# yifanlu0227/CoAlign

Hardware: AMD Instinct MI355X
Metric: frames_per_s_5agent_opv2v_synthetic (higher is better)
Workload: dtype f32 (3x3 convolutions: every operand rounded to 22 significant bits and split into two fp16 terms, the low term scaled by 2^10 and the weights by a per-output-channel power of two so that both terms are normal fp16 numbers at any scale; three fp16 matrix products per fp32 product, f32 accumulation

## Files before the change

### coalign_amd/csrc/conv3x3_sp_s2.hip

```cpp
#include "common.h"

namespace {

typedef float floatx16 __attribute__((ext_vector_type(16)));
typedef _Float16 halfx8 __attribute__((ext_vector_type(8)));
typedef __attribute__((address_space(3))) void *lptr_t;

constexpr int kCoutTile = 64;
constexpr int TH = 4, TW = 32;
constexpr int PR = 2 * TH + 1;
constexpr int CPP = 34, ROWP = 2 * CPP;
constexpr int PIX = PR * ROWP, PIXP = (PIX + 63) / 64 * 64, PINS = PIXP / 64;
constexpr int WQ = 9 * 2 * 2 * kCoutTile, WINS = WQ / 64;
constexpr int W_BYTES = WQ * 16, B_BYTES = 4 * PIXP * 16;
constexpr int kMaxCout = 1024, kMaxCoutSkip = 512;
constexpr size_t OPERAND_BYTES = 2 * (size_t)W_BYTES + 2 * (size_t)B_BYTES, LDS_BYTES = OPERAND_BYTES + 2 * kMaxCout * sizeof(float);
constexpr int WAVES = 8, THREADS = 64 * WAVES;
constexpr int WJ = 5, PJ = 2, OPS = WJ + 4 * PJ;
static_assert(LDS_BYTES <= 160 * 1024, "LDS budget");
static_assert(PINS == 10 && WINS == 36, "the piece schedule below is written for 10 patch and 36 weight instructions");

struct S2Args {
    const uint4 *__restrict__ x;
    const unsigned long long *__restrict__ stamps;
    const int *__restrict__ tag_ptr;
    unsigned sparse_rows;
    const uint4 *__restrict__ wt, *__restrict__ zero;
    const float *__restrict__ bias, *__restrict__ wscale;
    uint4 *__restrict__ y;
    const uint4 *__restrict__ ws;
    const float *__restrict__ ws_scale;
    float *__restrict__ yskip;
    int *range_flag;
    int N, Cin, Cout, H, W, Ho, Wo, relu, tiles_x, tiles_y, total_tasks;
    int ablate;
#ifdef COALIGN_LAB
    long long *trace;
#endif
};

#ifdef COALIGN_LAB
#define S2_STAMP(k) if (a.trace && (g == 0 || g == 100) && lane == 0 && L < 64) a.trace[((((g ? 1 : 0) * 8 + wave) * 64) + L) * 4 + (k)] = (long long)__builtin_amdgcn_s_memtime()
#else
#define S2_STAMP(k)
#endif

__device__ __forceinline__ void swap32(unsigned &a, unsigned &b) {
    const auto q = __builtin_amdgcn_permlane32_swap(a, b, false, false);
    const unsigned x = q[0], y = q[1];
    a = x;
    b = y;
}

__device__ __forceinline__ void dma16(const uint4 *src, unsigned lds_byte) {
    asm volatile("s_mov_b32 m0, %0\n\ts_nop 0\n\tglobal_load_lds_dwordx4 %1, off" ::"s"(__builtin_amdgcn_readfirstlane(lds_byte)), "v"(src) : "memory", "m0");
}

struct Task {
    int cg, n, oy0, ox0;
};

struct Plan {
    int off[PJ];
    const uint4 *wsrc;
};

template <bool SPARSE, bool SKIP>
__global__ __launch_bounds__(THREADS, 2) void conv3x3_sp_s2_kernel(const S2Args a) {
    extern __shared__ __attribute__((aligned(1024))) char lds[];
    const int tid = threadIdx.x, wave = __builtin_amdgcn_readfirstlane(tid >> 6), lane = tid & 63, half = lane >> 5, p = lane & 31;
    const int HW = a.H * a.W, HWo = a.Ho * a.Wo, CI16 = a.Cin / 16, CO16 = a.Cout / 16, groups = a.Cout / kCoutTile, chunks = CI16;
    const unsigned lds0 = (unsigned)(size_t)(lptr_t)lds;
    const int bx = wave & 3, cq = wave >> 2;
    const int oyl = p >> 3, oxl = bx * 8 + (p & 7);
    int boff[9];
#pragma unroll
    for (int s = 0; s < 9; ++s) {
        const int dy = s / 3, dx = s % 3;
        boff[s] = 2 * half * PIXP + (2 * oyl + dy) * ROWP + (dx & 1) * CPP + oxl + (dx >> 1);
    }
    const int wlane = half * kCoutTile + cq * 32 + p;
    const unsigned tag = SPARSE ? (unsigned)*a.tag_ptr : 0u;
    float *lds_par = reinterpret_cast<float *>(lds + OPERAND_BYTES);
    for (int i = tid; i < a.Cout / 4; i += THREADS) {
        reinterpret_cast<float4 *>(lds_par)[i] = reinterpret_cast<const float4 *>(a.bias)[i];
        reinterpret_cast<float4 *>(lds_par + a.Cout)[i] = reinterpret_cast<const float4 *>(a.wscale)[i];
        if constexpr (SKIP) reinterpret_cast<float4 *>(lds_par + 2 * a.Cout)[i] = reinterpret_cast<const float4 *>(a.ws_scale)[i];
    }
    auto skip_w = [&](int cg, int c, uint4 (&w)[2]) {
        const uint4 *base = a.ws + ((size_t)(cg * chunks + c) * 4 + half) * kCoutTile + cq * 32 + p;
        w[0] = base[0];
        w[1] = base[2 * kCoutTile];
    };

    auto decode = [&](int t) {
        Task c;
        c.cg = t % groups;
        const int sp = t / groups, ty = sp / a.tiles_x;
        c.ox0 = (sp - ty * a.tiles_x) * TW;
        c.n = ty / a.tiles_y;
        c.oy0 = (ty - c.n * a.tiles_y) * TH;
        return c;
    };
    auto position = [&](const Task &t, int j, int &iy, int &ix) {
        const int ins = j == 0 ? wave : 8 + wave;
        const int i = ins * 64 + lane, r = i / ROWP, rem = i - r * ROWP, cp = rem >= CPP ? 1 : 0, k = rem - cp * CPP;
        iy = 2 * t.oy0 - 1 + r;
        ix = 2 * t.ox0 - 1 + 2 * k + cp;
        return (j == 0 || wave < 2) && i < PIX && k < (cp ? TW : TW + 1) && iy >= 0 && iy < a.H && ix >= 0 && ix < a.W;
    };
    auto make_plan_dense = [&](const Task &t) {
        Plan pl;
        pl.wsrc = a.wt + (size_t)t.cg * chunks * WQ + lane;
#pragma unroll
        for (int j = 0; j < PJ; ++j) {
            int iy, ix;
            const bool ok = position(t, j, iy, ix);
            pl.off[j] = ok ? t.n * CI16 * 4 * HW + iy * a.W + ix : -1;
        }
        return pl;
    };
    struct Stamps {
        unsigned long long st[PJ];
    };
    auto load_stamps = [&](const Task &t) {
        Stamps s;
#pragma unroll
        for (int j = 0; j < PJ; ++j) {
            int iy, ix;
            const bool ok = position(t, j, iy, ix);
            s.st[j] = 0ull;
            if (ok) s.st[j] = a.stamps[((size_t)t.n * a.H + iy) * a.W + ix];
        }
        return s;
    };
    auto make_plan_sparse = [&](const Task &t, const Stamps &s) {
        Plan pl;
        pl.wsrc = a.wt + (size_t)t.cg * chunks * WQ + lane;
#pragma unroll
        for (int j = 0; j < PJ; ++j) {
            const unsigned row = (unsigned)s.st[j];
            const bool ok = (unsigned)(s.st[j] >> 32) == tag && tag != 0u && row < a.sparse_rows;
            pl.off[j] = ok ? (int)(row * (unsigned)(CI16 * 4)) : -1;
        }
        return pl;
    };
    auto issue_op = [&](const Plan &pl, int c, int slot, int k) {
        if (k < WJ) {
            const bool ok = wave < 2 ? k < 3 : true;
            const int piece = wave < 2 ? 3 * wave + k : 6 + 5 * (wave - 2) + k;
            if (ok && !(a.ablate & 1)) dma16(pl.wsrc + (size_t)c * WQ + piece * 64, lds0 + slot * W_BYTES + piece * 1024);
        } else {
            const int j = (k - WJ) / 4, q = (k - WJ) % 4, ins = j == 0 ? wave : 8 + wave;
            if ((j == 0 || wave < 2) && !(a.ablate & 2)) {
                const uint4 *src = pl.off[j] < 0 ? a.zero : SPARSE ? a.x + (size_t)pl.off[j] + (c * 4 + q) : a.x + (size_t)pl.off[j] + ((size_t)c * 4 + q) * HW;
                dma16(src, lds0 + 2 * W_BYTES + slot * B_BYTES + (q * PIXP + ins * 64) * 16);
            }
        }
    };
    auto issue_all = [&](const Plan &pl, int c, int slot) {
#pragma unroll
        for (int k = 0; k < OPS; ++k) issue_op(pl, c, slot, k);
    };

    const int n_wg = gridDim.x;
    int g = blockIdx.x;
    {
        const int q = n_wg >> 3, r = n_wg & 7, k = g & 7, j = g >> 3;
        g = k * q + (k < r ? k : r) + j;
    }
    const int n_local = ((a.total_tasks - g + n_wg - 1) / n_wg) * chunks;
    if (n_local <= 0) return;
    int task = g;
    Task cur = decode(task);
    Plan plan;
    if constexpr (SPARSE) plan = make_plan_sparse(cur, load_stamps(cur));
    else plan = make_plan_dense(cur);
    issue_all(plan, 0, 0);
    if (wave >= WAVES / 2) __builtin_amdgcn_s_setprio(1);
    uint4 sw_cur[2] = {}, sw_nxt[2] = {};
    if constexpr (SKIP) skip_w(cur.cg, 0, sw_nxt);
    int L = 0;
    while (L < n_local) {
        const int oy = cur.oy0 + oyl, ox = cur.ox0 + oxl;
        const bool live = oy < a.Ho && ox < a.Wo;
        const bool wave_live = __builtin_amdgcn_readfirstlane((int)(cur.ox0 + bx * 8 < a.Wo)) != 0;
        const size_t pix = live ? (size_t)oy * a.Wo + ox : 0;
        floatx16 acc = {0}, accl = {0}, sacc = {0}, saccl = {0};
        Task next = cur;
        Plan nplan = plan;
        int ntask = task;
        Stamps nst;
#pragma unroll
        for (int j = 0; j < PJ; ++j) nst.st[j] = 0ull;
        for (int chunk = 0; chunk < chunks; ++chunk, ++L) {
            S2_STAMP(0);
            __builtin_amdgcn_s_waitcnt(0);
            S2_STAMP(1);
            __syncthreads();
            S2_STAMP(2);
            if constexpr (SKIP) {
#pragma unroll
                for (int t = 0; t < 2; ++t) {
                    asm volatile("" : "+v"(sw_nxt[t].x), "+v"(sw_nxt[t].y), "+v"(sw_nxt[t].z), "+v"(sw_nxt[t].w));
                    sw_cur[t] = sw_nxt[t];
                }
            }
            const bool more = L + 1 < n_local;
            int nc = chunk + 1;
            if constexpr (SPARSE) {
                if (chunk == chunks - 2 && L + 2 < n_local) {
                    ntask = task + n_wg;
                    next = decode(ntask);
                    nst = load_stamps(next);
                }
            }
            if (more && nc == chunks) {
                nc = 0;
                if constexpr (SPARSE) {
                    nplan = make_plan_sparse(next, nst);
                } else {
                    ntask = task + n_wg;
                    next = decode(ntask);
                    nplan = make_plan_dense(next);
                }
            }
            if constexpr (SKIP) {
                if (more) skip_w(nc == 0 ? next.cg : cur.cg, nc, sw_nxt);
            }
            const int slot_cur = L & 1, slot_next = (L + 1) & 1;
            if (wave_live && !(a.ablate & 4)) {
                const uint4 *bq = reinterpret_cast<const uint4 *>(lds + 2 * W_BYTES + slot_cur * B_BYTES), *wq = reinterpret_cast<const uint4 *>(lds + slot_cur * W_BYTES) + wlane;
                auto load_b = [&](int s, halfx8 (&b)[2]) {
#pragma unroll
                    for (int t = 0; t < 2; ++t) b[t] = __builtin_bit_cast(halfx8, bq[t * PIXP + boff[s]]);
                };
                auto load_w = [&](int s, halfx8 (&w)[2]) {
#pragma unroll
                    for (int t = 0; t < 2; ++t) w[t] = __builtin_bit_cast(halfx8, wq[((s * 2 + t) * 2) * kCoutTile]);
                };
                halfx8 bc[2], wc[2];
                load_b(0, bc);
                load_w(0, wc);
#pragma unroll
                for (int s = 0; s < 9; ++s) {
                    if (!(a.ablate & 16)) {
                        if (s == 0) __builtin_amdgcn_s_setprio(2);
                        if (s == 3) __builtin_amdgcn_s_setprio(1);
                        if (s == 6) __builtin_amdgcn_s_setprio(0);
                    }
                    halfx8 bn[2], wn[2];
                    if (s + 1 < 9) {
                        load_b(s + 1, bn);
                        load_w(s + 1, wn);
                    }
                    accl = __builtin_amdgcn_mfma_f32_32x32x16_f16(wc[0], bc[1], accl, 0, 0, 0);
                    acc = __builtin_amdgcn_mfma_f32_32x32x16_f16(wc[0], bc[0], acc, 0, 0, 0);
                    accl = __builtin_amdgcn_mfma_f32_32x32x16_f16(wc[1], bc[0], accl, 0, 0, 0);
                    if constexpr (SKIP) {
                        if (s == 4) {
                            const halfx8 sh = __builtin_bit_cast(halfx8, sw_cur[0]), sl = __builtin_bit_cast(halfx8, sw_cur[1]);
                            saccl = __builtin_amdgcn_mfma_f32_32x32x16_f16(sh, bc[1], saccl, 0, 0, 0);
                            sacc = __builtin_amdgcn_mfma_f32_32x32x16_f16(sh, bc[0], sacc, 0, 0, 0);
                            saccl = __builtin_amdgcn_mfma_f32_32x32x16_f16(sl, bc[0], saccl, 0, 0, 0);
                        }
                    }
                    if (more) {
                        if (a.ablate & 32) {
#pragma unroll
                            for (int k = s; k < OPS; k += 9) issue_op(nplan, nc, slot_next, k);
                        } else {
#pragma unroll
                            for (int k = 2 * s; k < 2 * s + 2; ++k)
                                if (k < OPS) issue_op(nplan, nc, slot_next, k);
                        }
                    }
                    if (s + 1 < 9) {
#pragma unroll
                        for (int t = 0; t < 2; ++t) {
                            bc[t] = bn[t];
                            wc[t] = wn[t];
                        }
                    }
                }
            } else if (more) {
                issue_all(nplan, nc, slot_next);
            }
            S2_STAMP(3);
        }
#pragma unroll
        for (int e = 0; e < 16; ++e) acc[e] = fmaf(accl[e], coalign::kSp16LowInv, acc[e]);
        const int ch0 = cur.cg * kCoutTile + cq * 32 + 4 * half;
        const float4 *bias4 = reinterpret_cast<const float4 *>(lds_par + ch0), *winv4 = reinterpret_cast<const float4 *>(lds_par + a.Cout + ch0);
        const float floor_v = a.relu ? 0.f : -__builtin_inff();
        float vmax = 0.f;
        uint4 *ysp = a.y + ((size_t)(cur.n * CO16 + cur.cg * 4 + cq * 2) * 4 + half) * HWo + pix;
        const size_t sp_step = 2 * (size_t)HWo;
#pragma unroll
        for (int g8 = 0; g8 < 4; ++g8) {
            const float4 b4 = bias4[2 * g8], i4 = winv4[2 * g8];
            const float bb[4] = {b4.x, b4.y, b4.z, b4.w}, ii[4] = {i4.x, i4.y, i4.z, i4.w};
            float v[4];
#pragma unroll
            for (int j = 0; j < 4; ++j) v[j] = fmaxf(acc[4 * g8 + j] * ii[j] + (0.f + bb[j]), floor_v);
            vmax = fmaxf(fmaxf(fabsf(v[0]), fabsf(v[1])), fmaxf(fmaxf(fabsf(v[2]), fabsf(v[3])), vmax));
            unsigned h01, l01, h23, l23;
            coalign::sp16_split2(v[0], v[1], h01, l01);
            coalign::sp16_split2(v[2], v[3], h23, l23);
            swap32(h01, l01);
            swap32(h23, l23);
            if (live && wave_live && !(a.ablate & 8)) *ysp = uint4{h01, h23, l01, l23};
            ysp += sp_step;
        }
        if (a.range_flag && live && wave_live && vmax > 65504.f) atomicOr(a.range_flag, 1);
        if constexpr (SKIP) {
            const float4 *sinv4 = reinterpret_cast<const float4 *>(lds_par + 2 * a.Cout + ch0);
            float4 *ys = reinterpret_cast<float4 *>(a.yskip + ((size_t)cur.n * HWo + pix) * a.Cout + ch0);
#pragma unroll
            for (int g8 = 0; g8 < 4; ++g8) {
                const float4 i4 = sinv4[2 * g8];
                float4 o;
                o.x = fmaf(saccl[4 * g8], coalign::kSp16LowInv, sacc[4 * g8]) * i4.x;
                o.y = fmaf(saccl[4 * g8 + 1], coalign::kSp16LowInv, sacc[4 * g8 + 1]) * i4.y;
                o.z = fmaf(saccl[4 * g8 + 2], coalign::kSp16LowInv, sacc[4 * g8 + 2]) * i4.z;
                o.w = fmaf(saccl[4 * g8 + 3], coalign::kSp16LowInv, sacc[4 * g8 + 3]) * i4.w;
                if (live && wave_live && !(a.ablate & 8)) ys[2 * g8] = o;
            }
        }
        cur = next;
        plan = nplan;
        task = ntask;
    }
}

__global__ void sp_pack_rows_kernel(const float *__restrict__ rows, uint4 *__restrict__ out, int M, const int *__restrict__ count_ptr, int C, int *range_flag) {
    const size_t i = (size_t)blockIdx.x * blockDim.x + threadIdx.x;
    const int G8 = C / 8;
    if (count_ptr) M = min(max(*count_ptr, 0), M);
    if (i >= (size_t)M * G8) return;
    const int g8 = (int)(i % G8);
    const size_t row = i / G8;
    const float4 *src = reinterpret_cast<const float4 *>(rows + row * C + 8 * g8);
    const float4 q0 = src[0], q1 = src[1];
    const float v[8] = {q0.x, q0.y, q0.z, q0.w, q1.x, q1.y, q1.z, q1.w};
    unsigned h[4], l[4];
    bool big = false;
#pragma unroll
    for (int k = 0; k < 4; ++k) {
        coalign::sp16_split2(v[2 * k], v[2 * k + 1], h[k], l[k]);
        big = big || fabsf(v[2 * k]) > 65504.f || fabsf(v[2 * k + 1]) > 65504.f;
    }
    const size_t base = row * (size_t)(C / 16 * 4) + (size_t)(g8 / 2) * 4 + (g8 % 2) * 2;
    out[base] = uint4{h[0], h[1], h[2], h[3]};
    out[base + 1] = uint4{l[0], l[1], l[2], l[3]};
    if (range_flag && big) atomicOr(range_flag, 1);
}

#ifdef COALIGN_LAB
long long *g_s2_trace = nullptr;
#endif

int s2_check(int N, int Cin, int Cout, int H, int W) {
    if (N < 0 || H < 1 || W < 1 || Cin < 1 || Cout < 1) return COALIGN_ERR_BAD_SHAPE;
    if (Cin % 16 || Cout % kCoutTile || Cout > kMaxCout) return COALIGN_ERR_UNSUPPORTED;
    if ((int64_t)N * (Cin > Cout ? Cin : Cout) * H * W > (int64_t)1 << 32) return COALIGN_ERR_UNSUPPORTED;
    return COALIGN_OK;
}

template <bool SPARSE, bool SKIP>
int launch_s2(S2Args a, hipStream_t s) {
    constexpr int kMaxDev = 16;
    static int cus[kMaxDev] = {0};
    int dev = 0;
    if (hipGetDevice(&dev) != hipSuccess || dev < 0 || dev >= kMaxDev) dev = 0;
    auto kern = conv3x3_sp_s2_kernel<SPARSE, SKIP>;
    if (!cus[dev]) {
        hipDeviceProp_t prop;
        if (hipGetDeviceProperties(&prop, dev) != hipSuccess || prop.multiProcessorCount <= 0) prop.multiProcessorCount = 256;
        const int rc = coalign::hip_call(hipFuncSetAttribute(reinterpret_cast<const void *>(kern), hipFuncAttributeMaxDynamicSharedMemorySize, (int)LDS_BYTES));
        if (rc != COALIGN_OK) {
            (void)hipGetLastError();
            return rc;
        }
        cus[dev] = prop.multiProcessorCount;
    }
    a.Ho = (a.H + 1) / 2;
    a.Wo = (a.W + 1) / 2;
    a.tiles_x = (a.Wo + TW - 1) / TW;
    a.tiles_y = (a.Ho + TH - 1) / TH;
    a.total_tasks = a.tiles_x * a.tiles_y * a.N * (a.Cout / kCoutTile);
    const int rounds = (a.total_tasks + cus[dev] - 1) / cus[dev], grid = (a.total_tasks + rounds - 1) / rounds;
    hipLaunchKernelGGL(kern, dim3(grid), dim3(THREADS), LDS_BYTES, s, a);
    return coalign::check_launch();
}

int fill_common(S2Args &a, const void *w_split, const float *bias, void *y_sp, int N, int Cin, int Cout, int H, int W, int relu, int32_t *range_flag) {
    const size_t wbytes = coalign_conv3x3_emu_weight_bytes_ex(Cin, Cout, 16, 1), tail = (size_t)Cout * 8;
    const char *wb = static_cast<const char *>(w_split);
    a.wt = static_cast<const uint4 *>(w_split);
    a.zero = reinterpret_cast<const uint4 *>(wb + wbytes - tail - 16);
    a.bias = bias;
    a.wscale = reinterpret_cast<const float *>(wb + wbytes - tail);
    a.y = static_cast<uint4 *>(y_sp);
    a.range_flag = range_flag;
    a.N = N; a.Cin = Cin; a.Cout = Cout; a.H = H; a.W = W; a.relu = relu;
#ifdef COALIGN_LAB
    a.trace = g_s2_trace;
#endif
    a.ablate = coalign::lab_env("COALIGN_S2_ABLATE", 0);
    return COALIGN_OK;
}

}

#ifdef COALIGN_LAB
extern "C" void coalign_conv3x3_sp_s2_set_trace(long long *p) { g_s2_trace = p; }
#endif

extern "C" size_t coalign_sp_rows_bytes(int M, int C) {
    if (M < 0 || C < 16 || C % 16) return 0;
    return (size_t)M * C * 4;
}

extern "C" int coalign_sp_pack_rows(const float *rows, int M_capacity, const int32_t *M_dev, int C, void *rows_sp, int32_t *range_flag, void *stream) {
    if (!rows || !rows_sp) return COALIGN_ERR_NULL_POINTER;
    if (M_capacity < 0 || C < 16) return COALIGN_ERR_BAD_SHAPE;
    if (C % 16 || ((reinterpret_cast<uintptr_t>(rows) | reinterpret_cast<uintptr_t>(rows_sp)) & 15)) return COALIGN_ERR_UNSUPPORTED;
    const size_t n = (size_t)M_capacity * (C / 8);
    if (n == 0) return COALIGN_OK;
    hipLaunchKernelGGL(sp_pack_rows_kernel, dim3((unsigned)((n + 255) / 256)), dim3(256), 0, static_cast<hipStream_t>(stream), rows, static_cast<uint4 *>(rows_sp), M_capacity, M_dev, C,
                       range_flag);
    return coalign::check_launch();
}

extern "C" int coalign_conv3x3_sp_s2(const void *x_sp, const void *w_split, const float *bias, void *y_sp, int N, int Cin, int Cout, int H, int W, int relu,
                                     int32_t *range_flag, void *stream) {
    if (!x_sp || !w_split || !bias || !y_sp) return COALIGN_ERR_NULL_POINTER;
    int rc = s2_check(N, Cin, Cout, H, W);
    if (rc != COALIGN_OK) return rc;
    if ((reinterpret_cast<uintptr_t>(x_sp) | reinterpret_cast<uintptr_t>(w_split) | reinterpret_cast<uintptr_t>(y_sp) | reinterpret_cast<uintptr_t>(bias)) & 15) return COALIGN_ERR_UNSUPPORTED;
    if (N == 0) return COALIGN_OK;
    S2Args a{};
    a.x = static_cast<const uint4 *>(x_sp);
    fill_common(a, w_split, bias, y_sp, N, Cin, Cout, H, W, relu, range_flag);
    return launch_s2<false, false>(a, static_cast<hipStream_t>(stream));
}

extern "C" int coalign_conv3x3_sp_s2_sparse(const void *rows_sp, int M_rows, const void *stamps, const int32_t *state, const void *w_split, const float *bias, void *y_sp,
                                            int N, int Cin, int Cout, int H, int W, int relu, int32_t *range_flag, void *stream) {
    if (!rows_sp || !stamps || !state || !w_split || !bias || !y_sp) return COALIGN_ERR_NULL_POINTER;
    if (M_rows < 0) return COALIGN_ERR_BAD_SHAPE;
    int rc = s2_check(N, Cin, Cout, H, W);
    if (rc != COALIGN_OK) return rc;
    if (Cin < 32) return COALIGN_ERR_UNSUPPORTED;
    if ((reinterpret_cast<uintptr_t>(rows_sp) | reinterpret_cast<uintptr_t>(w_split) | reinterpret_cast<uintptr_t>(y_sp) | reinterpret_cast<uintptr_t>(bias)) & 15) return COALIGN_ERR_UNSUPPORTED;
    if (reinterpret_cast<uintptr_t>(stamps) & 7) return COALIGN_ERR_UNSUPPORTED;
    if ((int64_t)M_rows * Cin / 4 >= (int64_t)1 << 31) return COALIGN_ERR_UNSUPPORTED;
    if (N == 0) return COALIGN_OK;
    S2Args a{};
    a.x = static_cast<const uint4 *>(rows_sp);
    a.stamps = static_cast<const unsigned long long *>(stamps);
    a.tag_ptr = state;
    a.sparse_rows = (unsigned)M_rows;
    fill_common(a, w_split, bias, y_sp, N, Cin, Cout, H, W, relu, range_flag);
    return launch_s2<true, false>(a, static_cast<hipStream_t>(stream));
}

extern "C" size_t coalign_conv1x1_sp_weight_bytes(int Cin, int Cout) {
    if (Cin < 16 || Cin % 16 || Cout < kCoutTile || Cout % kCoutTile) return 0;
    return (size_t)Cout * Cin * 4 + 16 + (size_t)Cout * 8;
}

static int fill_skip(S2Args &a, const void *w_skip, float *y_skip, int Cin, int Cout) {
    if (!w_skip || !y_skip) return COALIGN_ERR_NULL_POINTER;
    if (Cout > kMaxCoutSkip || ((reinterpret_cast<uintptr_t>(w_skip) | reinterpret_cast<uintptr_t>(y_skip)) & 15)) return COALIGN_ERR_UNSUPPORTED;
    a.ws = static_cast<const uint4 *>(w_skip);
    a.ws_scale = reinterpret_cast<const float *>(static_cast<const char *>(w_skip) + (size_t)Cout * Cin * 4 + 16);
    a.yskip = y_skip;
    return COALIGN_OK;
}

extern "C" int coalign_conv3x3_sp_s2_skip(const void *x_sp, const void *w_split, const float *bias, const void *w_skip, void *y_sp, float *y_skip, int N, int Cin, int Cout, int H, int W,
                                          int relu, int32_t *range_flag, void *stream) {
    if (!x_sp || !w_split || !bias || !y_sp) return COALIGN_ERR_NULL_POINTER;
    int rc = s2_check(N, Cin, Cout, H, W);
    if (rc != COALIGN_OK) return rc;
    if ((reinterpret_cast<uintptr_t>(x_sp) | reinterpret_cast<uintptr_t>(w_split) | reinterpret_cast<uintptr_t>(y_sp) | reinterpret_cast<uintptr_t>(bias)) & 15) return COALIGN_ERR_UNSUPPORTED;
    S2Args a{};
    rc = fill_skip(a, w_skip, y_skip, Cin, Cout);
    if (rc != COALIGN_OK) return rc;
    if (N == 0) return COALIGN_OK;
    a.x = static_cast<const uint4 *>(x_sp);
    fill_common(a, w_split, bias, y_sp, N, Cin, Cout, H, W, relu, range_flag);
    return launch_s2<false, true>(a, static_cast<hipStream_t>(stream));
}

extern "C" int coalign_conv3x3_sp_s2_skip_sparse(const void *rows_sp, int M_rows, const void *stamps, const int32_t *state, const void *w_split, const float *bias, const void *w_skip,
                                                 void *y_sp, float *y_skip, int N, int Cin, int Cout, int H, int W, int relu, int32_t *range_flag, void *stream) {
    if (!rows_sp || !stamps || !state || !w_split || !bias || !y_sp) return COALIGN_ERR_NULL_POINTER;
    if (M_rows < 0) return COALIGN_ERR_BAD_SHAPE;
    int rc = s2_check(N, Cin, Cout, H, W);
    if (rc != COALIGN_OK) return rc;
    if (Cin < 32) return COALIGN_ERR_UNSUPPORTED;
    if ((reinterpret_cast<uintptr_t>(rows_sp) | reinterpret_cast<uintptr_t>(w_split) | reinterpret_cast<uintptr_t>(y_sp) | reinterpret_cast<uintptr_t>(bias)) & 15) return COALIGN_ERR_UNSUPPORTED;
    if (reinterpret_cast<uintptr_t>(stamps) & 7) return COALIGN_ERR_UNSUPPORTED;
    if ((int64_t)M_rows * Cin / 4 >= (int64_t)1 << 31) return COALIGN_ERR_UNSUPPORTED;
    S2Args a{};
    rc = fill_skip(a, w_skip, y_skip, Cin, Cout);
    if (rc != COALIGN_OK) return rc;
    if (N == 0) return COALIGN_OK;
    a.x = static_cast<const uint4 *>(rows_sp);
    a.stamps = static_cast<const unsigned long long *>(stamps);
    a.tag_ptr = state;
    a.sparse_rows = (unsigned)M_rows;
    fill_common(a, w_split, bias, y_sp, N, Cin, Cout, H, W, relu, range_flag);
    return launch_s2<true, true>(a, static_cast<hipStream_t>(stream));
}
```

Baseline: 672.1.

## Pair adjacent tasks per work unit to share patch or weight loads

Groups two tasks into one work unit. They are either two Cout groups over the same spatial tile, which share the input patch, or two spatial tiles with a single Cout group, which share the weights. Per chunk, the second task's pass loads only the operand that differs, using independent weight and patch LDS slots. This cuts global-to-LDS traffic per MFMA. The cost is doubled accumulator registers, more barriers per chunk, and fewer work units, which can hurt load balance across CUs.

```diff
diff --git a/coalign_amd/csrc/conv3x3_sp_s2.hip b/coalign_amd/csrc/conv3x3_sp_s2.hip
--- a/coalign_amd/csrc/conv3x3_sp_s2.hip
+++ b/coalign_amd/csrc/conv3x3_sp_s2.hip
@@ -33,6 +33,7 @@
     float *__restrict__ yskip;
     int *range_flag;
     int N, Cin, Cout, H, W, Ho, Wo, relu, tiles_x, tiles_y, total_tasks;
+    int total_units, pairing;
     int ablate;
 #ifdef COALIGN_LAB
     long long *trace;
@@ -60,9 +61,14 @@
     int cg, n, oy0, ox0;
 };
 
+struct Unit {
+    Task t0, t1;
+    int paired;
+};
+
 struct Plan {
     int off[PJ];
-    const uint4 *wsrc;
+    const uint4 *wsrc, *ssrc;
 };
 
 template <bool SPARSE, bool SKIP>
@@ -87,8 +93,8 @@
         reinterpret_cast<float4 *>(lds_par + a.Cout)[i] = reinterpret_cast<const float4 *>(a.wscale)[i];
         if constexpr (SKIP) reinterpret_cast<float4 *>(lds_par + 2 * a.Cout)[i] = reinterpret_cast<const float4 *>(a.ws_scale)[i];
     }
-    auto skip_w = [&](int cg, int c, uint4 (&w)[2]) {
-        const uint4 *base = a.ws + ((size_t)(cg * chunks + c) * 4 + half) * kCoutTile + cq * 32 + p;
+    auto skip_w = [&](const uint4 *ssrc, int c, uint4 (&w)[2]) {
+        const uint4 *base = ssrc + (size_t)c * 4 * kCoutTile;
         w[0] = base[0];
         w[1] = base[2 * kCoutTile];
     };
@@ -102,6 +108,25 @@
         c.oy0 = (ty - c.n * a.tiles_y) * TH;
         return c;
     };
+    auto decode_unit = [&](int u) {
+        Unit un;
+        int t0 = u;
+        un.paired = 0;
+        if (a.pairing) {
+            if (groups == 1) {
+                t0 = 2 * u;
+                if (t0 + 1 < a.total_tasks) un.paired = 2;
+            } else {
+                const int ups = (groups + 1) >> 1, sp = u / ups, k = u - sp * ups;
+                t0 = sp * groups + 2 * k;
+                if (2 * k + 1 < groups) un.paired = 1;
+            }
+        }
+        un.t0 = decode(t0);
+        un.t1 = un.t0;
+        if (un.paired) un.t1 = decode(t0 + 1);
+        return un;
+    };
     auto position = [&](const Task &t, int j, int &iy, int &ix) {
         const int ins = j == 0 ? wave : 8 + wave;
         const int i = ins * 64 + lane, r = i / ROWP, rem = i - r * ROWP, cp = rem >= CPP ? 1 : 0, k = rem - cp * CPP;
@@ -109,9 +134,13 @@
         ix = 2 * t.ox0 - 1 + 2 * k + cp;
         return (j == 0 || wave < 2) && i < PIX && k < (cp ? TW : TW + 1) && iy >= 0 && iy < a.H && ix >= 0 && ix < a.W;
     };
+    auto weights_of = [&](const Task &t, Plan &pl) {
+        pl.wsrc = a.wt + (size_t)t.cg * chunks * WQ + lane;
+        pl.ssrc = SKIP ? a.ws + ((size_t)(t.cg * chunks) * 4 + half) * kCoutTile + cq * 32 + p : nullptr;
+    };
     auto make_plan_dense = [&](const Task &t) {
         Plan pl;
-        pl.wsrc = a.wt + (size_t)t.cg * chunks * WQ + lane;
+        weights_of(t, pl);
 #pragma unroll
         for (int j = 0; j < PJ; ++j) {
             int iy, ix;
@@ -136,7 +165,7 @@
     };
     auto make_plan_sparse = [&](const Task &t, const Stamps &s) {
         Plan pl;
-        pl.wsrc = a.wt + (size_t)t.cg * chunks * WQ + lane;
+        weights_of(t, pl);
 #pragma unroll
         for (int j = 0; j < PJ; ++j) {
             const unsigned row = (unsigned)s.st[j];
@@ -145,22 +174,34 @@
         }
         return pl;
     };
-    auto issue_op = [&](const Plan &pl, int c, int slot, int k) {
+    auto make_plans_dense = [&](const Unit &u, Plan (&pl)[2]) {
+        pl[0] = make_plan_dense(u.t0);
+        pl[1] = pl[0];
+        if (u.paired == 2) pl[1] = make_plan_dense(u.t1);
+        weights_of(u.t1, pl[1]);
+    };
+    auto make_plans_sparse = [&](const Unit &u, const Stamps (&st)[2], Plan (&pl)[2]) {
+        pl[0] = make_plan_sparse(u.t0, st[0]);
+        pl[1] = pl[0];
+        if (u.paired == 2) pl[1] = make_plan_sparse(u.t1, st[1]);
+        weights_of(u.t1, pl[1]);
+    };
+    auto issue_op = [&](const Plan &pl, int c, int wslot, int pslot, bool need_w, bool need_p, int k) {
         if (k < WJ) {
             const bool ok = wave < 2 ? k < 3 : true;
             const int piece = wave < 2 ? 3 * wave + k : 6 + 5 * (wave - 2) + k;
-            if (ok && !(a.ablate & 1)) dma16(pl.wsrc + (size_t)c * WQ + piece * 64, lds0 + slot * W_BYTES + piece * 1024);
+            if (ok && need_w && !(a.ablate & 1)) dma16(pl.wsrc + (size_t)c * WQ + piece * 64, lds0 + wslot * W_BYTES + piece * 1024);
         } else {
             const int j = (k - WJ) / 4, q = (k - WJ) % 4, ins = j == 0 ? wave : 8 + wave;
-            if ((j == 0 || wave < 2) && !(a.ablate & 2)) {
+            if ((j == 0 || wave < 2) && need_p && !(a.ablate & 2)) {
                 const uint4 *src = pl.off[j] < 0 ? a.zero : SPARSE ? a.x + (size_t)pl.off[j] + (c * 4 + q) : a.x + (size_t)pl.off[j] + ((size_t)c * 4 + q) * HW;
-                dma16(src, lds0 + 2 * W_BYTES + slot * B_BYTES + (q * PIXP + ins * 64) * 16);
+                dma16(src, lds0 + 2 * W_BYTES + pslot * B_BYTES + (q * PIXP + ins * 64) * 16);
             }
         }
     };
-    auto issue_all = [&](const Plan &pl, int c, int slot) {
-#pragma unroll
-        for (int k = 0; k < OPS; ++k) issue_op(pl, c, slot, k);
+    auto issue_all = [&](const Plan &pl, int c, int wslot, int pslot, bool need_w, bool need_p) {
+#pragma unroll
+        for (int k = 0; k < OPS; ++k) issue_op(pl, c, wslot, pslot, need_w, need_p, k);
     };
 
     const int n_wg = gridDim.x;
@@ -169,167 +210,209 @@
         const int q = n_wg >> 3, r = n_wg & 7, k = g & 7, j = g >> 3;
         g = k * q + (k < r ? k : r) + j;
     }
-    const int n_local = ((a.total_tasks - g + n_wg - 1) / n_wg) * chunks;
-    if (n_local <= 0) return;
-    int task = g;
-    Task cur = decode(task);
-    Plan plan;
-    if constexpr (SPARSE) plan = make_plan_sparse(cur, load_stamps(cur));
-    else plan = make_plan_dense(cur);
-    issue_all(plan, 0, 0);
+    if (g >= a.total_units) return;
+    int unit = g;
+    Unit cur = decode_unit(unit);
+    Plan pl[2];
+    if constexpr (SPARSE) {
+        Stamps st[2];
+        st[0] = load_stamps(cur.t0);
+        st[1] = st[0];
+        if (cur.paired == 2) st[1] = load_stamps(cur.t1);
+        make_plans_sparse(cur, st, pl);
+    } else {
+        make_plans_dense(cur, pl);
+    }
+    issue_all(pl[0], 0, 0, 0, true, true);
     if (wave >= WAVES / 2) __builtin_amdgcn_s_setprio(1);
     uint4 sw_cur[2] = {}, sw_nxt[2] = {};
-    if constexpr (SKIP) skip_w(cur.cg, 0, sw_nxt);
-    int L = 0;
-    while (L < n_local) {
-        const int oy = cur.oy0 + oyl, ox = cur.ox0 + oxl;
-        const bool live = oy < a.Ho && ox < a.Wo;
-        const bool wave_live = __builtin_amdgcn_readfirstlane((int)(cur.ox0 + bx * 8 < a.Wo)) != 0;
-        const size_t pix = live ? (size_t)oy * a.Wo + ox : 0;
-        floatx16 acc = {0}, accl = {0}, sacc = {0}, saccl = {0};
-        Task next = cur;
-        Plan nplan = plan;
-        int ntask = task;
-        Stamps nst;
-#pragma unroll
-        for (int j = 0; j < PJ; ++j) nst.st[j] = 0ull;
-        for (int chunk = 0; chunk < chunks; ++chunk, ++L) {
-            S2_STAMP(0);
-            __builtin_amdgcn_s_waitcnt(0);
-            S2_STAMP(1);
-            __syncthreads();
-            S2_STAMP(2);
+    if constexpr (SKIP) skip_w(pl[0].ssrc, 0, sw_nxt);
+    int L = 0, wslot = 0, pslot = 0;
+    for (;;) {
+        const bool has_next = unit + n_wg < a.total_units;
+        bool live[2], wave_live[2];
+        size_t pix[2];
+#pragma unroll
+        for (int i = 0; i < 2; ++i) {
+            const Task &tk = i ? cur.t1 : cur.t0;
+            const int oy = tk.oy0 + oyl, ox = tk.ox0 + oxl;
+            live[i] = oy < a.Ho && ox < a.Wo;
+            wave_live[i] = __builtin_amdgcn_readfirstlane((int)(tk.ox0 + bx * 8 < a.Wo)) != 0;
+            pix[i] = live[i] ? (size_t)oy * a.Wo + ox : 0;
+        }
+        floatx16 acc[2] = {{0}, {0}}, accl[2] = {{0}, {0}}, sacc[2] = {{0}, {0}}, saccl[2] = {{0}, {0}};
+        Unit next = cur;
+        Plan npl[2] = {pl[0], pl[1]};
+        Stamps nst[2];
+#pragma unroll
+        for (int j = 0; j < PJ; ++j) nst[0].st[j] = nst[1].st[j] = 0ull;
+        for (int chunk = 0; chunk < chunks; ++chunk) {
+#pragma unroll
+            for (int i = 0; i < 2; ++i) {
+                if (i == 1 && !cur.paired) continue;
+                S2_STAMP(0);
+                __builtin_amdgcn_s_waitcnt(0);
+                S2_STAMP(1);
+                __syncthreads();
+                S2_STAMP(2);
+                if constexpr (SKIP) {
+#pragma unroll
+                    for (int t = 0; t < 2; ++t) {
+                        asm volatile("" : "+v"(sw_nxt[t].x), "+v"(sw_nxt[t].y), "+v"(sw_nxt[t].z), "+v"(sw_nxt[t].w));
+                        sw_cur[t] = sw_nxt[t];
+                    }
+                }
+                if (i == 0 && has_next) {
+                    if constexpr (SPARSE) {
+                        if (chunk == chunks - 2) {
+                            next = decode_unit(unit + n_wg);
+                            nst[0] = load_stamps(next.t0);
+                            if (next.paired == 2) nst[1] = load_stamps(next.t1);
+                        }
+                        if (chunk == chunks - 1) make_plans_sparse(next, nst, npl);
+                    } else if (chunk == chunks - 1) {
+                        next = decode_unit(unit + n_wg);
+                        make_plans_dense(next, npl);
+                    }
+                }
+                bool more = true, need_w = true, need_p = true;
+                Plan np = pl[0];
+                int nc = chunk + 1;
+                if (i == 0 && cur.paired) {
+                    np = pl[1];
+                    nc = chunk;
+                    need_w = cur.paired == 1;
+                    need_p = cur.paired == 2;
+                } else if (nc == chunks) {
+                    more = has_next;
+                    np = npl[0];
+                    nc = 0;
+                }
+                if constexpr (SKIP) {
+                    if (more) skip_w(np.ssrc, nc, sw_nxt);
+                }
+                const int wnext = need_w ? wslot ^ 1 : wslot, pnext = need_p ? pslot ^ 1 : pslot;
+                if (wave_live[i] && !(a.ablate & 4)) {
+                    const uint4 *bq = reinterpret_cast<const uint4 *>(lds + 2 * W_BYTES + pslot * B_BYTES), *wq = reinterpret_cast<const uint4 *>(lds + wslot * W_BYTES) + wlane;
+                    auto load_b = [&](int s, halfx8 (&b)[2]) {
+#pragma unroll
+                        for (int t = 0; t < 2; ++t) b[t] = __builtin_bit_cast(halfx8, bq[t * PIXP + boff[s]]);
+                    };
+                    auto load_w = [&](int s, halfx8 (&w)[2]) {
+#pragma unroll
+                        for (int t = 0; t < 2; ++t) w[t] = __builtin_bit_cast(halfx8, wq[((s * 2 + t) * 2) * kCoutTile]);
+                    };
+                    halfx8 bc[2], wc[2];
+                    load_b(0, bc);
+                    load_w(0, wc);
+#pragma unroll
+                    for (int s = 0; s < 9; ++s) {
+                        if (!(a.ablate & 16)) {
+                            if (s == 0) __builtin_amdgcn_s_setprio(2);
+                            if (s == 3) __builtin_amdgcn_s_setprio(1);
+                            if (s == 6) __builtin_amdgcn_s_setprio(0);
+                        }
+                        halfx8 bn[2], wn[2];
+                        if (s + 1 < 9) {
+                            load_b(s + 1, bn);
+                            load_w(s + 1, wn);
+                        }
+                        accl[i] = __builtin_amdgcn_mfma_f32_32x32x16_f16(wc[0], bc[1], accl[i], 0, 0, 0);
+                        acc[i] = __builtin_amdgcn_mfma_f32_32x32x16_f16(wc[0], bc[0], acc[i], 0, 0, 0);
+                        accl[i] = __builtin_amdgcn_mfma_f32_32x32x16_f16(wc[1], bc[0], accl[i], 0, 0, 0);
+                        if constexpr (SKIP) {
+                            if (s == 4) {
+                                const halfx8 sh = __builtin_bit_cast(halfx8, sw_cur[0]), sl = __builtin_bit_cast(halfx8, sw_cur[1]);
+                                saccl[i] = __builtin_amdgcn_mfma_f32_32x32x16_f16(sh, bc[1], saccl[i], 0, 0, 0);
+                                sacc[i] = __builtin_amdgcn_mfma_f32_32x32x16_f16(sh, bc[0], sacc[i], 0, 0, 0);
+                                saccl[i] = __builtin_amdgcn_mfma_f32_32x32x16_f16(sl, bc[0], saccl[i], 0, 0, 0);
+                            }
+                        }
+                        if (more) {
+                            if (a.ablate & 32) {
+#pragma unroll
+                                for (int k = s; k < OPS; k += 9) issue_op(np, nc, wnext, pnext, need_w, need_p, k);
+                            } else if (need_w) {
+#pragma unroll
+                                for (int k = 2 * s; k < 2 * s + 2; ++k)
+                                    if (k < OPS) issue_op(np, nc, wnext, pnext, true, need_p, k);
+                            } else {
+#pragma unroll
+                                for (int k = WJ + 2 * s; k < WJ + 2 * s + 2; ++k)
+                                    if (k < OPS) issue_op(np, nc, wnext, pnext, false, true, k);
+                            }
+                        }
+                        if (s + 1 < 9) {
+#pragma unroll
+                            for (int t = 0; t < 2; ++t) {
+                                bc[t] = bn[t];
+                                wc[t] = wn[t];
+                            }
+                        }
+                    }
+                } else if (more) {
+                    issue_all(np, nc, wnext, pnext, need_w, need_p);
+                }
+                if (more) {
+                    wslot = wnext;
+                    pslot = pnext;
+                }
+                S2_STAMP(3);
+                ++L;
+            }
+        }
+        const float floor_v = a.relu ? 0.f : -__builtin_inff();
+        const size_t sp_step = 2 * (size_t)HWo;
+        float vmax = 0.f;
+#pragma unroll
+        for (int i = 0; i < 2; ++i) {
+            if (i == 1 && !cur.paired) continue;
+            const Task &tk = i ? cur.t1 : cur.t0;
+            const bool store = live[i] && wave_live[i] && !(a.ablate & 8);
+#pragma unroll
+            for (int e = 0; e < 16; ++e) acc[i][e] = fmaf(accl[i][e], coalign::kSp16LowInv, acc[i][e]);
+            const int ch0 = tk.cg * kCoutTile + cq * 32 + 4 * half;
+            const float4 *bias4 = reinterpret_cast<const float4 *>(lds_par + ch0), *winv4 = reinterpret_cast<const float4 *>(lds_par + a.Cout + ch0);
+            float vm = 0.f;
+            uint4 *ysp = a.y + ((size_t)(tk.n * CO16 + tk.cg * 4 + cq * 2) * 4 + half) * HWo + pix[i];
+#pragma unroll
+            for (int g8 = 0; g8 < 4; ++g8) {
+                const float4 b4 = bias4[2 * g8], i4 = winv4[2 * g8];
+                const float bb[4] = {b4.x, b4.y, b4.z, b4.w}, ii[4] = {i4.x, i4.y, i4.z, i4.w};
+                float v[4];
+#pragma unroll
+                for (int j = 0; j < 4; ++j) v[j] = fmaxf(acc[i][4 * g8 + j] * ii[j] + (0.f + bb[j]), floor_v);
+                vm = fmaxf(fmaxf(fabsf(v[0]), fabsf(v[1])), fmaxf(fmaxf(fabsf(v[2]), fabsf(v[3])), vm));
+                unsigned h01, l01, h23, l23;
+                coalign::sp16_split2(v[0], v[1], h01, l01);
+                coalign::sp16_split2(v[2], v[3], h23, l23);
+                swap32(h01, l01);
+                swap32(h23, l23);
+                if (store) *ysp = uint4{h01, h23, l01, l23};
+                ysp += sp_step;
+            }
+            if (live[i] && wave_live[i]) vmax = fmaxf(vmax, vm);
             if constexpr (SKIP) {
-#pragma unroll
-                for (int t = 0; t < 2; ++t) {
-                    asm volatile("" : "+v"(sw_nxt[t].x), "+v"(sw_nxt[t].y), "+v"(sw_nxt[t].z), "+v"(sw_nxt[t].w));
-                    sw_cur[t] = sw_nxt[t];
+                const float4 *sinv4 = reinterpret_cast<const float4 *>(lds_par + 2 * a.Cout + ch0);
+                float4 *ys = reinterpret_cast<float4 *>(a.yskip + ((size_t)tk.n * HWo + pix[i]) * a.Cout + ch0);
+#pragma unroll
+                for (int g8 = 0; g8 < 4; ++g8) {
+                    const float4 i4 = sinv4[2 * g8];
+                    float4 o;
+                    o.x = fmaf(saccl[i][4 * g8], coalign::kSp16LowInv, sacc[i][4 * g8]) * i4.x;
+                    o.y = fmaf(saccl[i][4 * g8 + 1], coalign::kSp16LowInv, sacc[i][4 * g8 + 1]) * i4.y;
+                    o.z = fmaf(saccl[i][4 * g8 + 2], coalign::kSp16LowInv, sacc[i][4 * g8 + 2]) * i4.z;
+                    o.w = fmaf(saccl[i][4 * g8 + 3], coalign::kSp16LowInv, sacc[i][4 * g8 + 3]) * i4.w;
+                    if (store) ys[2 * g8] = o;
                 }
             }
-            const bool more = L + 1 < n_local;
-            int nc = chunk + 1;
-            if constexpr (SPARSE) {
-                if (chunk == chunks - 2 && L + 2 < n_local) {
-                    ntask = task + n_wg;
-                    next = decode(ntask);
-                    nst = load_stamps(next);
-                }
-            }
-            if (more && nc == chunks) {
-                nc = 0;
-                if constexpr (SPARSE) {
-                    nplan = make_plan_sparse(next, nst);
-                } else {
-                    ntask = task + n_wg;
-                    next = decode(ntask);
-                    nplan = make_plan_dense(next);
-                }
-            }
-            if constexpr (SKIP) {
-                if (more) skip_w(nc == 0 ? next.cg : cur.cg, nc, sw_nxt);
-            }
-            const int slot_cur = L & 1, slot_next = (L + 1) & 1;
-            if (wave_live && !(a.ablate & 4)) {
-                const uint4 *bq = reinterpret_cast<const uint4 *>(lds + 2 * W_BYTES + slot_cur * B_BYTES), *wq = reinterpret_cast<const uint4 *>(lds + slot_cur * W_BYTES) + wlane;
-                auto load_b = [&](int s, halfx8 (&b)[2]) {
-#pragma unroll
-                    for (int t = 0; t < 2; ++t) b[t] = __builtin_bit_cast(halfx8, bq[t * PIXP + boff[s]]);
-                };
-                auto load_w = [&](int s, halfx8 (&w)[2]) {
-#pragma unroll
-                    for (int t = 0; t < 2; ++t) w[t] = __builtin_bit_cast(halfx8, wq[((s * 2 + t) * 2) * kCoutTile]);
-                };
-                halfx8 bc[2], wc[2];
-                load_b(0, bc);
-                load_w(0, wc);
-#pragma unroll
-                for (int s = 0; s < 9; ++s) {
-                    if (!(a.ablate & 16)) {
-                        if (s == 0) __builtin_amdgcn_s_setprio(2);
-                        if (s == 3) __builtin_amdgcn_s_setprio(1);
-                        if (s == 6) __builtin_amdgcn_s_setprio(0);
-                    }
-                    halfx8 bn[2], wn[2];
-                    if (s + 1 < 9) {
-                        load_b(s + 1, bn);
-                        load_w(s + 1, wn);
-                    }
-                    accl = __builtin_amdgcn_mfma_f32_32x32x16_f16(wc[0], bc[1], accl, 0, 0, 0);
-                    acc = __builtin_amdgcn_mfma_f32_32x32x16_f16(wc[0], bc[0], acc, 0, 0, 0);
-                    accl = __builtin_amdgcn_mfma_f32_32x32x16_f16(wc[1], bc[0], accl, 0, 0, 0);
-                    if constexpr (SKIP) {
-                        if (s == 4) {
-                            const halfx8 sh = __builtin_bit_cast(halfx8, sw_cur[0]), sl = __builtin_bit_cast(halfx8, sw_cur[1]);
-                            saccl = __builtin_amdgcn_mfma_f32_32x32x16_f16(sh, bc[1], saccl, 0, 0, 0);
-                            sacc = __builtin_amdgcn_mfma_f32_32x32x16_f16(sh, bc[0], sacc, 0, 0, 0);
-                            saccl = __builtin_amdgcn_mfma_f32_32x32x16_f16(sl, bc[0], saccl, 0, 0, 0);
-                        }
-                    }
-                    if (more) {
-                        if (a.ablate & 32) {
-#pragma unroll
-                            for (int k = s; k < OPS; k += 9) issue_op(nplan, nc, slot_next, k);
-                        } else {
-#pragma unroll
-                            for (int k = 2 * s; k < 2 * s + 2; ++k)
-                                if (k < OPS) issue_op(nplan, nc, slot_next, k);
-                        }
-                    }
-                    if (s + 1 < 9) {
-#pragma unroll
-                        for (int t = 0; t < 2; ++t) {
-                            bc[t] = bn[t];
-                            wc[t] = wn[t];
-                        }
-                    }
-                }
-            } else if (more) {
-                issue_all(nplan, nc, slot_next);
-            }
-            S2_STAMP(3);
-        }
-#pragma unroll
-        for (int e = 0; e < 16; ++e) acc[e] = fmaf(accl[e], coalign::kSp16LowInv, acc[e]);
-        const int ch0 = cur.cg * kCoutTile + cq * 32 + 4 * half;
-        const float4 *bias4 = reinterpret_cast<const float4 *>(lds_par + ch0), *winv4 = reinterpret_cast<const float4 *>(lds_par + a.Cout + ch0);
-        const float floor_v = a.relu ? 0.f : -__builtin_inff();
-        float vmax = 0.f;
-        uint4 *ysp = a.y + ((size_t)(cur.n * CO16 + cur.cg * 4 + cq * 2) * 4 + half) * HWo + pix;
-        const size_t sp_step = 2 * (size_t)HWo;
-#pragma unroll
-        for (int g8 = 0; g8 < 4; ++g8) {
-            const float4 b4 = bias4[2 * g8], i4 = winv4[2 * g8];
-            const float bb[4] = {b4.x, b4.y, b4.z, b4.w}, ii[4] = {i4.x, i4.y, i4.z, i4.w};
-            float v[4];
-#pragma unroll
-            for (int j = 0; j < 4; ++j) v[j] = fmaxf(acc[4 * g8 + j] * ii[j] + (0.f + bb[j]), floor_v);
-            vmax = fmaxf(fmaxf(fabsf(v[0]), fabsf(v[1])), fmaxf(fmaxf(fabsf(v[2]), fabsf(v[3])), vmax));
-            unsigned h01, l01, h23, l23;
-            coalign::sp16_split2(v[0], v[1], h01, l01);
-            coalign::sp16_split2(v[2], v[3], h23, l23);
-            swap32(h01, l01);
-            swap32(h23, l23);
-            if (live && wave_live && !(a.ablate & 8)) *ysp = uint4{h01, h23, l01, l23};
-            ysp += sp_step;
-        }
-        if (a.range_flag && live && wave_live && vmax > 65504.f) atomicOr(a.range_flag, 1);
-        if constexpr (SKIP) {
-            const float4 *sinv4 = reinterpret_cast<const float4 *>(lds_par + 2 * a.Cout + ch0);
-            float4 *ys = reinterpret_cast<float4 *>(a.yskip + ((size_t)cur.n * HWo + pix) * a.Cout + ch0);
-#pragma unroll
-            for (int g8 = 0; g8 < 4; ++g8) {
-                const float4 i4 = sinv4[2 * g8];
-                float4 o;
-                o.x = fmaf(saccl[4 * g8], coalign::kSp16LowInv, sacc[4 * g8]) * i4.x;
-                o.y = fmaf(saccl[4 * g8 + 1], coalign::kSp16LowInv, sacc[4 * g8 + 1]) * i4.y;
-                o.z = fmaf(saccl[4 * g8 + 2], coalign::kSp16LowInv, sacc[4 * g8 + 2]) * i4.z;
-                o.w = fmaf(saccl[4 * g8 + 3], coalign::kSp16LowInv, sacc[4 * g8 + 3]) * i4.w;
-                if (live && wave_live && !(a.ablate & 8)) ys[2 * g8] = o;
-            }
-        }
+        }
+        if (a.range_flag && vmax > 65504.f) atomicOr(a.range_flag, 1);
+        if (!has_next) break;
         cur = next;
-        plan = nplan;
-        task = ntask;
+        pl[0] = npl[0];
+        pl[1] = npl[1];
+        unit += n_wg;
     }
 }
 
@@ -388,8 +471,11 @@
     a.Wo = (a.W + 1) / 2;
     a.tiles_x = (a.Wo + TW - 1) / TW;
     a.tiles_y = (a.Ho + TH - 1) / TH;
-    a.total_tasks = a.tiles_x * a.tiles_y * a.N * (a.Cout / kCoutTile);
-    const int rounds = (a.total_tasks + cus[dev] - 1) / cus[dev], grid = (a.total_tasks + rounds - 1) / rounds;
+    const int groups = a.Cout / kCoutTile, tiles = a.tiles_x * a.tiles_y * a.N;
+    a.total_tasks = tiles * groups;
+    a.pairing = coalign::lab_env("COALIGN_S2_UNPAIRED", 0) ? 0 : 1;
+    a.total_units = !a.pairing ? a.total_tasks : groups == 1 ? (tiles + 1) / 2 : tiles * ((groups + 1) / 2);
+    const int rounds = (a.total_units + cus[dev] - 1) / cus[dev], grid = (a.total_units + rounds - 1) / rounds;
     hipLaunchKernelGGL(kern, dim3(grid), dim3(THREADS), LDS_BYTES, s, a);
     return coalign::check_launch();
 }
```

After: 669.2. No clear change (-0.4%).
